# seqan/sahara

Measured on AMD Instinct MI355X. Metric: reads/s at k=2 edit, 10M×100bp vs 3Gbp index; achieved HBM GB/s, higher is better.
Workload: dtype u32; 1 GPU; C3: k=2 lev, 10000000x100bp reads (+RC) per GPU vs 3 Gbp 24-record index, h2-k2; reads_per_gpu=10000000, read_len=100, errors=2, ref_len=3000000000, records=24, generator=h2-k2, searches=3, parallelism=replicated-index x1 (query shards), hits_total=25990613, build_id=7339ec07fe5cacd5

## Files before the change

### include/sahara_hip.h

```cpp
#ifndef SAHARA_HIP_H
#define SAHARA_HIP_H

#include <stddef.h>
#include <stdint.h>

#ifdef __cplusplus
extern "C" {
#endif

typedef struct sahara_hit {
    uint64_t qid;
    uint32_t seq_id;
    uint32_t err;
    uint64_t pos;
} sahara_hit;

typedef struct sahara_index_info {
    uint32_t sigma;
    uint32_t sampling_rate;
    uint64_t n;
    uint64_t n_records;
    uint64_t n_samples;
    uint64_t device_bytes;
    uint32_t n_parts;
// ... 20 lines not shown
    double   text_ms;
    uint64_t fm_iterations;
    uint64_t text_iterations;
    uint64_t text_active;
    uint64_t text_refills;
    uint64_t text_cycles_refill;
    uint64_t text_cycles_step;
    uint64_t text_cycles_emit;
    uint64_t text_compare_steps;
    uint32_t text_grid;
    uint32_t pipelined;
    double   seed_ms;
    uint64_t text_steps;
    double   stage_ms;
    double   output_ms;
    uint64_t text_launches;
    uint64_t upload_chunks[3];
    uint64_t text_pos_tasks;
    uint64_t text_stolen;
    uint64_t best_rounds;
    uint64_t best_skipped;
    uint64_t reserved[6];
} sahara_stats;

const char* sahara_gpu_last_error(void);
int  sahara_gpu_device_count(void);
const char* sahara_build_id(void);

int  sahara_gpu_open(int device, const void* idx_image, size_t idx_bytes, void** ctx);
int  sahara_gpu_open_file(int device, const char* idx_path, void** ctx);
int  sahara_gpu_build(int device, const uint8_t* ranks, const uint64_t* rec_lens, uint64_t n_records,
                      uint32_t sigma, uint32_t sampling_rate, void** ctx);
int  sahara_gpu_save(void* ctx, const char* path);
int  sahara_gpu_index_info(void* ctx, sahara_index_info* info);
int  sahara_gpu_export(void* ctx, uint8_t* bwt_f, uint8_t* bwt_r, uint64_t* sampled_bits,
                       uint32_t* samples, uint64_t* C, uint64_t* rec_lens);
int  sahara_gpu_export_sa(void* ctx, uint32_t* sa);
int  sahara_gpu_export_text(void* ctx, uint8_t* text);
int  sahara_gpu_select_part(void* ctx, uint32_t part);
int  sahara_gpu_part_info(void* ctx, uint32_t part, sahara_index_info* info);
int  sahara_gpu_set_mode(void* ctx, int verify, int locate_sa);

int  sahara_gpu_search(void* ctx, const uint8_t* ranks, uint64_t n_patterns, uint32_t len,
                       const uint32_t* pi, const uint32_t* l, const uint32_t* u, uint32_t n_searches,
                       int edit, uint32_t max_hits, sahara_hit** hits, uint64_t* n_hits);
int  sahara_gpu_search_reads(void* ctx, const uint8_t* reads, uint64_t n_reads, uint32_t len, int reverse,
// ... 189 lines not shown
```

### sahara_amd/__init__.py

```python
from __future__ import annotations

import ctypes as C
import os

import numpy as np

__all__ = [
    "BiFMIndex", "HIT_DTYPE", "search", "search_reads", "search_reads_compact", "CompactHits", "PackedReads",
    "pack_reads", "search_packed", "search_packed_compact", "search_best", "search_best_reads", "search_best_packed",
    "search_best_packed_compact", "ALIGN_DTYPE", "ALIGN_MAX_ERR", "ALIGN_NONE", "align", "align_packed_compact",
    "align_stats", "cigar", "PAIR_SUMMARY_DTYPE", "PAIR_NONE", "PAIR_LINK_DTYPE", "LINK_PRIMARY", "pair_mapq", "read_fasta", "search_scheme", "scheme_parts",
    "scheme_generators",
    "scheme_counts", "synth_reference", "synth_reads", "interleave_rc", "load_fasta",
    "library_path", "lib", "SaharaError", "DNA5", "DNA4",
]

_HERE = os.path.dirname(os.path.abspath(__file__))
_LIB = None

DNA5 = {"sigma": 6, "chars": "$ACGNT"}
DNA4 = {"sigma": 5, "chars": "$ACGT"}

HIT_DTYPE = np.dtype([("qid", "<u8"), ("seq_id", "<u4"), ("err", "<u4"), ("pos", "<u8")])
ALIGN_MAX_ERR = 8
# ... 25 lines not shown
class IndexInfo(C.Structure):
    _fields_ = [("sigma", C.c_uint32), ("sampling_rate", C.c_uint32), ("n", C.c_uint64),
                ("n_records", C.c_uint64), ("n_samples", C.c_uint64), ("device_bytes", C.c_uint64),
                ("n_parts", C.c_uint32), ("kmer_depth", C.c_uint32)]


class Stats(C.Structure):
    _fields_ = [("patterns", C.c_uint64), ("batches", C.c_uint64), ("cursors", C.c_uint64),
                ("hits", C.c_uint64), ("search_ms", C.c_double), ("locate_ms", C.c_double),
                ("sort_ms", C.c_double), ("total_ms", C.c_double), ("nodes", C.c_uint64),
                ("rank_nodes", C.c_uint64), ("ext_lines", C.c_uint64), ("lf_steps", C.c_uint64),
                ("search_launches", C.c_uint32), ("search_grid", C.c_uint32),
                ("text_nodes", C.c_uint64), ("conversions", C.c_uint64), ("text_ms", C.c_double),
                ("fm_iterations", C.c_uint64), ("text_iterations", C.c_uint64), ("text_active", C.c_uint64),
                ("text_refills", C.c_uint64), ("text_cycles_refill", C.c_uint64),
                ("text_cycles_step", C.c_uint64), ("text_cycles_emit", C.c_uint64),
                ("text_compare_steps", C.c_uint64), ("text_grid", C.c_uint32), ("pipelined", C.c_uint32),
                ("seed_ms", C.c_double), ("text_steps", C.c_uint64), ("stage_ms", C.c_double),
                ("output_ms", C.c_double), ("text_launches", C.c_uint64),
                ("upload_chunks", C.c_uint64 * 3), ("text_pos_tasks", C.c_uint64),
                ("text_stolen", C.c_uint64), ("best_rounds", C.c_uint64), ("best_skipped", C.c_uint64),
                ("reserved", C.c_uint64 * 6)]

    def as_dict(self):
        return {n: (list(v) if isinstance(v, C.Array) else v) for n, v in
                ((n, getattr(self, n)) for n, _ in self._fields_)}


class AlignStats(C.Structure):
    _fields_ = [("hits", C.c_uint64), ("chunks", C.c_uint64), ("kernel_ms", C.c_double), ("stage_ms", C.c_double),
                ("total_ms", C.c_double)]


class LociStats(C.Structure):
    _fields_ = [("hits_in", C.c_uint64), ("loci", C.c_uint64), ("batches", C.c_uint64), ("kernel_ms", C.c_double)]


class PairsStats(C.Structure):
    _fields_ = [("hits_in", C.c_uint64), ("kept", C.c_uint64), ("pairs", C.c_uint64), ("batches", C.c_uint64),
                ("kernel_ms", C.c_double)]


class BestPairsStats(C.Structure):
    _fields_ = [("hits_in", C.c_uint64), ("kept", C.c_uint64), ("pairs", C.c_uint64), ("unique_pairs", C.c_uint64),
                ("batches", C.c_uint64), ("kernel_ms", C.c_double)]


PAIR_SUMMARY_DTYPE = np.dtype([("best", "u1"), ("next", "u1"), ("n_fwd", "<u2"), ("n_rev", "<u2"), ("reserved", "<u2")])
PAIR_NONE = 255
# ... 832 lines not shown
```

### sahara_amd/csrc/pass.cpp

```cpp
#include <algorithm>
#include <cstdlib>
#include <chrono>
#include <thread>

#include <sys/prctl.h>

#include "ctx.h"
#include "align_core.h"
#include "best_pairs_core.h"
#include "rescue_core.h"

namespace sahara {

DeviceIndex& partOf(Ctx* c, uint32_t p) { return p == 0 ? c->I : c->more.at(p - 1); }

void checkPairsCall(const Ctx* c, uint64_t npat, uint32_t len) {
    if (c->rescue.on) {
        if (!c->pairs.on) throw Error("rescue: needs pairs on (a mate is looked for in the pair rule's fragment window)");
        if (len > kAlignMaxLen)
            throw Error("rescue: the pattern length " + std::to_string(len) + " is above " + std::to_string(kAlignMaxLen));
        if (c->pairs.maxFrag >= len) {
            const PairDist d = pairDist(len, c->pairs.minFrag, c->pairs.maxFrag);
            if (d.dmax - d.dmin >= kRescueMaxWindow)
                throw Error("rescue: the fragment window of " + std::to_string(d.dmax - d.dmin + 1) +
// ... 41 lines not shown
                if (p) std::swap(c->I, c->more[p - 1]);
            });
            runOne(c, count);
        }
        if (c->outAll.cap < total + c->nout)
            c->outAll.growKeeping(std::max<uint64_t>((total + c->nout) + (total + c->nout) / 4, 1024), total, c->st);
        launchOffsetSeq(c->out.ptr, c->nout, c->partRec0[p], c->outAll.ptr + total, c->st);
        total += c->nout;
        const sahara_stats& S = c->stats;
        T.patterns = S.patterns;
        T.search_grid = S.search_grid;
        T.text_grid = S.text_grid;
        T.pipelined = S.pipelined;
        T.best_rounds = S.best_rounds;
        for (uint64_t sahara_stats::*f :
             {&sahara_stats::batches, &sahara_stats::cursors, &sahara_stats::nodes, &sahara_stats::rank_nodes,
              &sahara_stats::ext_lines, &sahara_stats::lf_steps, &sahara_stats::text_nodes,
              &sahara_stats::conversions, &sahara_stats::fm_iterations, &sahara_stats::text_iterations,
              &sahara_stats::text_active, &sahara_stats::text_refills, &sahara_stats::text_cycles_refill,
              &sahara_stats::text_cycles_step, &sahara_stats::text_cycles_emit, &sahara_stats::text_compare_steps,
              &sahara_stats::text_steps, &sahara_stats::text_launches,
              &sahara_stats::text_pos_tasks, &sahara_stats::text_stolen, &sahara_stats::best_skipped})
            T.*f += S.*f;
        for (double sahara_stats::*f : {&sahara_stats::search_ms, &sahara_stats::locate_ms, &sahara_stats::sort_ms,
                                        &sahara_stats::text_ms, &sahara_stats::seed_ms})
            T.*f += S.*f;
        T.search_launches += S.search_launches;
    }
    if (c->out.cap < total) {
        c->out.release();
        c->out.reserve(std::max<uint64_t>(total, 1024));
    }
    sortHitsByQid(c->outAll.ptr, total, c->npat, c->out.ptr, c->merge, c->tmp, c->st);
    SH_HIP(hipStreamSynchronize(c->st));
    c->sk.done = 0;
    c->nout = total;
    T.hits = total;
    T.total_ms = std::chrono::duration<double, std::milli>(std::chrono::steady_clock::now() - t0).count();
    T.stage_ms = c->stageMs;
    for (int b = 0; b < 3; ++b) T.upload_chunks[b] = c->stats.upload_chunks[b];
    c->stats = T;
}

void runOne(Ctx* c, bool count) {
    if (!c->sk.staged) throw Error("sahara_gpu_run: nothing staged");
    auto t0 = std::chrono::steady_clock::now();
// ... 184 lines not shown
    t.text3Bytes = (uint32_t)std::min<uint64_t>(text3Blocks(c->I.n) * 16, 0xFFFFFF00ull);
    t.pats3Bytes = (uint32_t)std::min<uint64_t>((P.bstart[b + 1] - q0) * c->patBlocks * 16, 0xFFFFFF00ull);
    t.m = c->m;
    t.nsearch = R.nsearch;
    t.table = reinterpret_cast<const uint2*>(c->cover.ptr + R.coverAt);
    t.tasks = sl.tasks.ptr;
    t.taskCount = sl.small.ptr + kSwTaskCount;
    t.taskBegin = r ? sl.small.ptr + kSwRoundTasks : nullptr;
    t.taskCap = c->taskCap;
    t.work = sl.queues.ptr + kQueueSeedTasks;
    t.hits = sl.hits.ptr;
    t.hitCap = c->hitCap;
    t.hitCount = sl.small.ptr + kSwHitCount;
    t.filled = sl.small.ptr + kSwFilled;
    t.flags = sl.small.ptr + kSwFlags;
    t.counters = c->counters.ptr;
    t.winBlocks = P.tx.winBlocks;
    t.exactWindow = P.tx.exactWindow ? 1u : 0u;
    t.stackCap = P.tx.textStack;
    t.tableWords = P.tx.tableWords;
    t.steps = P.k.textSteps;
    t.refillAt = P.k.refillAt;
    t.stealAt = P.k.stealAt;
    t.qcnt = sl.qcnt.ptr;
    t.rank = sl.rank.ptr;
    t.probe = P.probe ? 1u : 0u;
    t.isFirst = b == 0 && r == 0 ? 1u : 0u;
    return t;
}

enum : uint32_t { kLocFlags = 2, kLocSegCounts = 4 };

static LocateArgs locateArgs(Ctx* c, Ctx::Slot& sl, uint64_t nhits) {
    LocateArgs la{};
    la.hits = sl.hits.ptr;
    la.nhits = nhits;
    la.qoff = c->qoff.ptr;
    la.rank = sl.rank.ptr;
    la.occF = c->I.occF.ptr;
    for (int i = 0; i < 8; ++i) la.C[i] = (uint32_t)c->I.C[i];
    la.samples = c->I.samples.ptr;
    la.rate = c->I.rate;
    la.keys = c->k0.ptr;
    la.flags = c->small.ptr + kLocFlags;
    la.counters = c->counters.ptr + kCtLfSteps;
    la.sa = c->I.saFull.ptr;
// ... 351 lines not shown
            *total += ms;
            if (s == kStagePairs) c->stageStats.pairs.pairs += c->pinned.ptr[b].pairs;
            if (s == kStagePairs && c->pairs.linksOn && c->pairs.bufs.linkTimed) {
                SH_HIP(hipEventElapsedTime(&ms, c->pairs.bufs.linkStart, c->pairs.bufs.linkDone));
                c->stageStats.linkMs += ms;
            }
        }
        c->mark("checked", b);
    }
};

static void readCounters(Ctx* c, const PassPlan& P, sahara_stats& S, hipStream_t sC) {
    unsigned long long h[kCounters];
    auto per = [&](Counter sum, Counter n) { return (double)h[sum] / std::max(1.0, (double)h[n]); };
    if (P.probe) {
        SH_HIP(hipMemcpy(h, c->counters.ptr, sizeof(h), hipMemcpyDeviceToHost));
        auto since = [&](Counter i) { return (h[i] - h[kCtBornMin]) / 100.0; };
        std::fprintf(stderr, "text wave lives (first launch, us): last start %.1f first end %.1f last end %.1f mean %.1f; "
                     "tasks all taken seen first %.1f last %.1f by %llu waves, which ran on %.1f on average\n",
                     since(kCtBornMax), since(kCtEndMin), since(kCtEndMax),
                     h[kCtLifeSum] / 100.0 / std::max<double>(1, S.text_grid * 4.0), since(kCtDryMin), since(kCtDryMax),
                     h[kCtDryWaves], per(kCtDryRun, kCtDryWaves) / 100.0);
        std::fprintf(stderr, "text iterations before / after: %llu (busy lanes %.1f) / %llu (busy lanes %.1f); "
                     "nodes stolen %llu\n",
                     h[kCtIterPre], per(kCtActPre, kCtIterPre), h[kCtIterPost], per(kCtActPost, kCtIterPost), h[kCtStolen]);
        std::fprintf(stderr, "text wall per iteration (us) before: refill %.2f steps+emit %.2f; after: refill %.2f steps+emit %.2f\n",
                     per(kCtWallPreRefill, kCtIterPre) / 100.0, per(kCtWallPreStep, kCtIterPre) / 100.0,
                     per(kCtWallPostRefill, kCtIterPost) / 100.0, per(kCtWallPostStep, kCtIterPost) / 100.0);
    }
    SH_HIP(hipMemcpyAsync(h, c->counters.ptr, sizeof(h), hipMemcpyDeviceToHost, sC));
    SH_HIP(hipStreamSynchronize(sC));
    static const std::pair<uint64_t sahara_stats::*, Counter> statOf[] = {
        {&sahara_stats::nodes, kCtNodes}, {&sahara_stats::rank_nodes, kCtRankNodes},
        {&sahara_stats::ext_lines, kCtExtLines}, {&sahara_stats::lf_steps, kCtLfSteps},
        {&sahara_stats::text_nodes, kCtTextNodes}, {&sahara_stats::conversions, kCtTextTasks},
        {&sahara_stats::fm_iterations, kCtFmIter}, {&sahara_stats::text_iterations, kCtTextIter},
        {&sahara_stats::text_active, kCtTextActive}, {&sahara_stats::text_refills, kCtTextRefills},
        {&sahara_stats::text_cycles_refill, kCtCyRefill}, {&sahara_stats::text_cycles_step, kCtCyStep},
        {&sahara_stats::text_cycles_emit, kCtCyEmit}, {&sahara_stats::text_compare_steps, kCtCompareSteps},
        {&sahara_stats::text_steps, kCtTextSteps}, {&sahara_stats::text_pos_tasks, kCtPosTasks},
        {&sahara_stats::text_stolen, kCtStolen}, {&sahara_stats::best_skipped, kCtBestSkipped}};
    for (const auto& so : statOf) S.*so.first = h[so.second];
    if (P.k.dump) {
        for (uint32_t i = 0; i < kCounters; ++i) std::fprintf(stderr, "%s%llu", i ? " " : "counters ", h[i]);
        std::fprintf(stderr, "\n");
    }
}

void runPass(Ctx* c, bool count, bool redo, sahara_stats& S, bool& overflow) {
    const PassPlan P = makePlan(c, count, redo);
    const uint64_t nbatch = P.nbatch();
    overflow = false;
    S.patterns = c->npat;
    S.search_grid = P.blocks;
    S.text_grid = P.split ? P.textBlocks : 0u;
    S.pipelined = P.serial ? 0u : 1u;
    S.best_rounds = P.rounds > 1 ? P.rounds : 0u;
    c->stack.reserve((size_t)P.stackLevels * std::max(P.blocks, P.firstBlocks) * 256);
    initWorkCaps(c, P.maxBatch, P.k);
    c->pinned.reserve(nbatch);
    reserveLocate(c, P.maxBatch, Ctx::kSlots);
    for (auto& sl : c->slot) SH_HIP(hipMemsetAsync(sl.qcnt.ptr, 0, (P.maxBatch + 1) * sizeof(uint32_t), c->st));
    Pass ps{c, P, S, overflow, c->st, P.serial ? c->st : c->stB, P.serial ? c->st : c->stC, P.serial ? c->st : c->stD};
    auto syncAll = [&](std::initializer_list<hipStream_t> ss) {
        for (hipStream_t s : ss) SH_HIP(hipStreamSynchronize(s));
// ... 73 lines not shown
```

### sahara_amd/csrc/pass_plan.h

```cpp
#pragma once
#include <algorithm>
#include <cstdint>
#include <cstdlib>
#include <optional>
#include <vector>

#include "fm_step.h"

namespace sahara {

constexpr uint32_t kTextTableMin = 3u * 256u;

inline std::vector<uint64_t> parseRamp(const char* e) {
    std::vector<uint64_t> v;
    for (const char* p = e; p && *p;) {
        char* end = nullptr;
        const unsigned long long x = std::strtoull(p, &end, 10);
        if (end == p) break;
        if (x) v.push_back(x);
        p = (*end == ',' || *end == ':') ? end + 1 : end;
    }
    return v;
}

struct PassKnobs {
    bool pipeline, dump, chunkSeeds, kmerPos, seedTasks;
    uint32_t fmLdsDepth, fmStealAt, stealAt, split, textSteps, refillAt, pollUs;
    uint32_t hitCap, taskCap;
    unsigned long timerSlackNs;
    std::optional<long> batch, fmBpc, textBpc;
    std::vector<uint64_t> rampHead, rampTail;
};

inline PassKnobs readPassKnobs(bool verify) {
    auto num = [](const char* name) -> std::optional<long> {
        const char* e = std::getenv(name);
        return e ? std::optional<long>(std::atol(e)) : std::nullopt;
    };
    auto within = [](long lo, long v, long hi) { return std::max(lo, std::min(hi, v)); };
    PassKnobs k{};
    k.pipeline = num("SAHARA_PIPELINE").value_or(1) != 0;
    k.dump = std::getenv("SAHARA_DUMP_COUNTERS") != nullptr;
    k.fmLdsDepth = (uint32_t)within(0, num("SAHARA_FM_LDS_DEPTH").value_or(verify ? 0 : 4), 8);
    k.fmStealAt = (uint32_t)within(0, num("SAHARA_FM_STEAL_AT").value_or(verify ? 0 : 8), 64);
    k.stealAt = (uint32_t)within(0, num("SAHARA_STEAL_AT").value_or(8), 64);
    k.split = (uint32_t)std::max(0L, num("SAHARA_SPLIT").value_or(1));
    k.textSteps = (uint32_t)std::max(1L, num("SAHARA_TEXT_STEPS").value_or(2));
    k.refillAt = (uint32_t)within(1, num("SAHARA_REFILL_AT").value_or(8), 64);
    k.chunkSeeds = num("SAHARA_CHUNK_SEEDS").value_or(1) != 0;
    k.kmerPos = num("SAHARA_KMER_POS").value_or(1) != 0;
    k.seedTasks = num("SAHARA_SEED_TASKS").value_or(1) != 0;
    k.pollUs = (uint32_t)std::max(0L, num("SAHARA_POLL_US").value_or(20));
    k.timerSlackNs = (unsigned long)std::max(0L, num("SAHARA_TIMER_SLACK_NS").value_or(1000));
    if (auto v = num("SAHARA_HITCAP")) k.hitCap = (uint32_t)std::max(1L, *v);
    if (auto v = num("SAHARA_TASKCAP")) k.taskCap = (uint32_t)std::max(1L, *v);
    k.batch = num("SAHARA_BATCH");
    k.fmBpc = num("SAHARA_FM_BPC");
    k.textBpc = num("SAHARA_TEXT_BPC");
    k.rampHead = parseRamp(std::getenv("SAHARA_RAMP"));
    k.rampTail = parseRamp(std::getenv("SAHARA_RAMP_END"));
    return k;
}

inline uint64_t maxBatchOf(std::optional<long> batch, bool streaming, uint32_t nsearch, bool compactRecs,
                           uint64_t granularity = 1) {
    const uint64_t most = (1ull << 31) / nsearch;
    uint64_t mb = std::min<uint64_t>(streaming ? 1ull << 21 : 1ull << 22, most);
    if (batch) mb = std::max<uint64_t>(1, std::min<uint64_t>(most, (uint64_t)*batch));
// ... 94 lines not shown
```

### sahara_amd/csrc/search.h

```cpp
#pragma once
#include <hip/hip_runtime.h>

#include <cstddef>
#include <cstdint>

#include "../../include/sahara_hip.h"
#include "device_index.h"

namespace sahara {

struct SearchArgs {
    const OccLine* occF;
    const OccLine* occR;
    uint32_t C[8];
    uint32_t n;
    const uint32_t* pats;
    uint32_t patWords;
    uint32_t m;
    uint32_t nsearch;
    uint32_t nitems;
    const uint4* seeds;
    const uint32_t* seedItem;
    const uint32_t* seedCount;
    const uint32_t* scheme;
// ... 63 lines not shown
    uint64_t rows;
    uint32_t nbig, nhuge;
    uint64_t kept;
    uint64_t pairs;
};
static_assert(sizeof(BatchRecord) == 64 && offsetof(BatchRecord, slot) == 0 &&
              offsetof(BatchRecord, locateFlags) == 4 * 7 && offsetof(BatchRecord, rows) == 4 * kSlotWords &&
              offsetof(BatchRecord, nbig) == 4 * 10 && offsetof(BatchRecord, nhuge) == 4 * 11 &&
              offsetof(BatchRecord, kept) == 4 * 12, "BatchRecord is what kBatchTotals and the batch's stages write");

constexpr uint32_t kCounters = 56;
enum Counter : uint32_t {
    kCtNodes = 0, kCtRankNodes = 1, kCtExtLines = 2, kCtLfSteps = 3, kCtDigest = 4, kCtTextNodes = 5,
    kCtTextTasks = 6, kCtFmIter = 7, kCtTextIter = 8, kCtTextActive = 9, kCtTextRefills = 10,
    kCtCyRefill = 11, kCtCyStep = 12, kCtCyEmit = 13,
    kCtCompareSteps = 14, kCtTextSteps = 15,
    kCtPosTasks = 16,
    kCtBestSkipped = 17,
    kCtDryRun = 30, kCtDryWaves = 31,
    kCtBornMin = 33, kCtBornMax = 34, kCtEndMax = 35, kCtLifeSum = 36, kCtEndMin = 37,
    kCtDryMin = 38, kCtDryMax = 39,
    kCtIterPre = 40, kCtActPre = 41, kCtIterPost = 42, kCtActPost = 43,
    kCtStolen = 45,
    kCtWallPreRefill = 46, kCtWallPreStep = 47, kCtWallPostRefill = 48, kCtWallPostStep = 49
};
struct TextBatchArgs {
    const uint32_t* sa;
    const uint4* text3;
    const uint4* pats3;
    uint32_t patBlocks;
    uint32_t text3Bytes;
    uint32_t pats3Bytes;
    uint32_t m;
    uint32_t nsearch;
    const uint2* table;
    const uint4* tasks;
    const uint32_t* taskCount;
    const uint32_t* taskBegin;
    uint32_t taskCap;
    uint32_t* work;
    uint4* hits;
    uint32_t hitCap;
    uint32_t* hitCount;
    uint32_t* filled;
    uint32_t* flags;
    unsigned long long* counters;
    uint32_t winBlocks;
    uint32_t exactWindow;
    uint32_t stackCap;
    uint32_t tableWords;
    uint32_t steps;
    uint32_t refillAt;
    uint32_t stealAt;
    uint32_t* qcnt;
    uint32_t* rank;
    uint32_t probe;
    uint32_t isFirst;
};

struct LocateArgs {
    const uint4* hits;
    uint64_t nhits;
    const uint64_t* qoff;
    const uint32_t* rank;
    const OccLine* occF;
    uint32_t C[8];
    const uint32_t* samples;
    uint32_t rate;
    uint64_t* keys;
    uint32_t* flags;
    unsigned long long* counters;
    const uint32_t* sa;
    uint32_t useSA;
};

int searchBlocksPerCU(uint32_t sigma, bool edit, size_t lds);
// ... 123 lines not shown
```

### sahara_amd/csrc/search_device.h

```cpp
#pragma once
#include <hip/hip_runtime.h>

#include "search.h"

namespace sahara {
namespace {

#if defined(__HIP_DEVICE_COMPILE__)
#define GLOB(T, p) ((__attribute__((address_space(1))) T*)(p))
#else
#define GLOB(T, p) ((T*)(p))
#endif
typedef uint32_t U32x4 __attribute__((ext_vector_type(4)));
__device__ __forceinline__ uint4 loadGlobal4(const uint4* p) {
    const U32x4 v = *GLOB(const U32x4, p);
    return make_uint4(v.x, v.y, v.z, v.w);
}

constexpr uint32_t kSeedChunk = 64;
constexpr uint32_t kTaskChunk = 64;
static_assert(kTaskChunk >= 1 && kTaskChunk <= 64, "a chunk's records sit one per lane");
constexpr uint32_t kHitChunk = 64;

struct SlotRange {
    uint32_t next = 0, end = 0;
// ... 54 lines not shown
        __builtin_amdgcn_wave_barrier();
    }
};
__device__ __forceinline__ StealPlan stealPlan(bool thief, bool canGive, uint32_t stealAt, uint32_t lane,
                                               uint64_t ltMask) {
    const uint64_t I = __ballot(thief);
    const uint64_t D = __ballot(canGive);
    const uint32_t nI = (uint32_t)__popcll(I), nD = (uint32_t)__popcll(D);
    if (nI < stealAt || !nD) return {false, false, false, lane};
    const uint32_t n = min(nI, nD);
    const uint32_t r = (uint32_t)__popcll(I & ltMask);
    uint32_t donor = 0, rr = r;
    uint64_t dm = D;
#pragma unroll
    for (uint32_t w = 32; w; w >>= 1) {
        const uint32_t c = (uint32_t)__popcll(dm & ((1ull << w) - 1ull));
        if (rr >= c) { rr -= c; dm >>= w; donor += w; }
    }
    const bool takes = thief && r < n;
    const bool gives = ((D >> lane) & 1ull) && (uint32_t)__popcll(D & ltMask) < n;
    return {true, takes, gives, takes ? donor : lane};
}

constexpr uint32_t kLdsStarts = 256;
template <typename Starts>
__device__ __forceinline__ sahara_hit decodeKey(uint64_t k, uint64_t qid, const Starts& starts, uint32_t nrec) {
    const uint64_t gpos = k >> 4;
    uint32_t lo = 0, hi = nrec;
    while (hi - lo > 1) {
        const uint32_t mid = (lo + hi) >> 1;
        if (starts[mid] <= gpos) lo = mid; else hi = mid;
    }
    sahara_hit h;
    h.qid = qid;
    h.seq_id = lo;
    h.err = (uint32_t)(k & 15u);
    h.pos = gpos - starts[lo];
    return h;
}

struct HitLess {
    __host__ __device__ bool operator()(const sahara_hit& a, const sahara_hit& b) const {
        if (a.qid != b.qid) return a.qid < b.qid;
        if (a.seq_id != b.seq_id) return a.seq_id < b.seq_id;
        if (a.pos != b.pos) return a.pos < b.pos;
        return a.err < b.err;
// ... 6 lines not shown
```

### sahara_amd/csrc/search_text.hip

```cpp

#include <hip/hip_runtime.h>

#include "fm_step.h"
#include "search_device.h"
#include "text_step.h"

namespace sahara {
namespace {

__device__ __forceinline__ uint32_t read32(const uint32_t* A, int o, uint32_t b) {
    const int i = o >> 5;
    return __builtin_amdgcn_alignbit(A[(3 * i + 3 + (int)b) * 256], A[(3 * i + (int)b) * 256], (uint32_t)o & 31u);
}
__device__ __forceinline__ Planes chain32(const uint32_t* A, uint32_t o, bool fwd) {
    const int off = (int)o - (fwd ? 0 : 32);
    Planes r;
    uint32_t v[3];
#pragma unroll
    for (uint32_t b = 0; b < 3; ++b) {
        const uint32_t w = read32(A, off, b);
        v[b] = fwd ? w : __builtin_bitreverse32(w);
    }
    r.b0 = v[0]; r.b1 = v[1]; r.b2 = v[2];
    return r;
// ... 157 lines not shown
    const StealPlan p = stealPlan(!ln.have && ln.sp == 0u, ln.sp >= 2u || (ln.sp == 1u && ln.have), stealAt, lane, ltMask);
    if (!p.any) return false;
    const uint32_t dPid = __shfl(ln.pid, p.donor), dWb = __shfl(ln.wb, p.donor), dBase = __shfl(ln.sBase, p.donor);
    const uint32_t dTid = (threadIdx.x & ~63u) | p.donor;
    if (p.takes) {
        const uint32_t* src = L.slot + dTid;
        uint32_t* dst = L.slot + threadIdx.x;
        for (uint32_t k = 0; k < L.copyWords(); ++k) dst[k * 256u] = src[k * 256u];
        const uint2 node = reinterpret_cast<const uint2*>(L.slot + L.copyWords() * 256u)[dTid];
        ln.cur = {node.x, node.y};
        ln.pid = dPid;
        ln.wb = dWb;
        ln.sBase = dBase;
        ln.have = true;
    }
    p.settle();
    if (p.gives) {
        for (uint32_t d = 1; d < ln.sp; ++d) L.stackPut(d - 1u, L.stackGet(d));
        --ln.sp;
    }
    return p.takes;
}

struct HitWriter {
    SlotRange slots;
    uint32_t rankSlot = ~0u, rankVal = 0;
    uint32_t filled = 0;
    __device__ __forceinline__ void emit(const TextBatchArgs& a, bool leaf, uint32_t lane, uint64_t ltMask, uint32_t pid,
                                         uint32_t pos, uint32_t e) {
        uint32_t s;
        if (slots.take(leaf, lane, ltMask, a.hitCount, s) && leaf) {
            if (s < a.hitCap) {
                a.hits[s] = make_uint4(pid, pos, 1u, e | kPosKnown);
                if (rankSlot != ~0u) a.rank[rankSlot] = rankVal;
                rankVal = atomicAdd(a.qcnt + pid, 1u);
                rankSlot = s;
            } else {
                atomicOr(a.flags, kFlagHits);
            }
            ++filled;
        }
    }
    __device__ __forceinline__ void finish(const TextBatchArgs& a, uint32_t lane) {
        slots.close(lane, a.hits, a.hitCap);
        if (rankSlot != ~0u) a.rank[rankSlot] = rankVal;
        if (filled) atomicAdd(a.filled, filled);
    }
};

template <bool COUNT>
struct TextProbe {
    __device__ __forceinline__ TextProbe(const TextBatchArgs&, uint32_t, uint64_t*) {}
    __device__ __forceinline__ void iterBegin() {}
    __device__ __forceinline__ void refilled(bool, bool, bool) {}
    __device__ __forceinline__ void stolen(bool) {}
    __device__ __forceinline__ void stepped(const TextStepResult&) {}
    __device__ __forceinline__ void stepsDone() {}
    __device__ __forceinline__ void emitted(bool) {}
    __device__ __forceinline__ void flush() {}
};
template <>
struct TextProbe<true> {
    const TextBatchArgs& a;
    const uint32_t lane;
    const bool wall;
    uint64_t* born;
    uint64_t cNodes = 0, cCmp = 0, cSteps = 0, cSteal = 0;
    uint64_t tIter = 0, tActive = 0, tRefill = 0;
    uint64_t cyRefill = 0, cyStep = 0, cyEmit = 0, t0 = 0;
    uint32_t pIterPre = 0, pIterPost = 0, pActPre = 0, pActPost = 0;
    uint64_t pwPreA = 0, pwPreB = 0, pwPostA = 0, pwPostB = 0, pw0 = 0, pw1 = 0;

    __device__ __forceinline__ TextProbe(const TextBatchArgs& args, uint32_t l, uint64_t* waveClock)
        : a(args), lane(l), wall(args.probe != 0u), born(waveClock + 2u * (threadIdx.x >> 6)) {
        if (wall && lane == 0) born[0] = wall_clock64(), born[1] = 0;
    }
    __device__ __forceinline__ void iterBegin() {
        if (wall) pw0 = wall_clock64();
        t0 = clock64();
    }
    __device__ __forceinline__ void refilled(bool qDone, bool active, bool refill) {
        const uint32_t act = (uint32_t)__popcll(__ballot(active));
        if (wall) {
            if (qDone && lane == 0 && born[1] == 0) born[1] = wall_clock64();
            if (qDone) { ++pIterPost; pActPost += act; } else { ++pIterPre; pActPre += act; }
            pw1 = wall_clock64();
        }
        if (lane == 0) { ++tIter; tActive += act; tRefill += refill ? 1u : 0u; }
        const uint64_t t1 = clock64();
        cyRefill += t1 - t0;
        t0 = t1;
    }
    __device__ __forceinline__ void stolen(bool took) { cSteal += took ? 1u : 0u; }
    __device__ __forceinline__ void stepped(const TextStepResult& r) {
        cNodes += r.nodes;
        cCmp += r.compares;
        cSteps += r.steps;
    }
    __device__ __forceinline__ void stepsDone() {
        const uint64_t t1 = clock64();
        cyStep += t1 - t0;
        t0 = t1;
    }
    __device__ __forceinline__ void emitted(bool qDone) {
        cyEmit += clock64() - t0;
        if (wall) {
            const uint64_t pw2 = wall_clock64();
            if (qDone) { pwPostA += pw1 - pw0; pwPostB += pw2 - pw1; }
            else { pwPreA += pw1 - pw0; pwPreB += pw2 - pw1; }
        }
    }
    __device__ __forceinline__ void add(uint32_t counter, uint64_t v) {
        atomicAdd(a.counters + counter, (unsigned long long)v);
    }
    __device__ __forceinline__ void flush() {
        if (wall && a.isFirst && lane == 0) {
// ... 10 lines not shown
                add(kCtDryWaves, 1);
            }
            add(kCtIterPre, pIterPre);
            add(kCtActPre, pActPre);
            add(kCtIterPost, pIterPost);
            add(kCtActPost, pActPost);
            add(kCtWallPreRefill, pwPreA);
            add(kCtWallPreStep, pwPreB);
            add(kCtWallPostRefill, pwPostA);
            add(kCtWallPostStep, pwPostB);
        }
        add(kCtTextNodes, cNodes);
        if (lane == 0) {
            add(kCtTextIter, tIter);
            add(kCtTextActive, tActive);
            add(kCtTextRefills, tRefill);
            add(kCtCyRefill, cyRefill);
            add(kCtCyStep, cyStep);
            add(kCtCyEmit, cyEmit);
        }
        add(kCtCompareSteps, cCmp);
        add(kCtTextSteps, cSteps);
        if (cSteal) add(kCtStolen, cSteal);
    }
};

template <bool EDIT, bool COUNT, int SHAPE>
__global__ __launch_bounds__(256) void kSearchTextBatch(TextBatchArgs a) {
    extern __shared__ uint32_t lds[];
    uint2* SC = reinterpret_cast<uint2*>(lds);
    for (uint32_t i = threadIdx.x; i < a.nsearch * a.m; i += blockDim.x) SC[i] = a.table[i];
    __syncthreads();

    const uint32_t lane = threadIdx.x & 63u;
    const uint64_t ltMask = (1ull << lane) - 1ull;
    constexpr TextShape kShape = textShape(SHAPE);
    LaneLds L;
    L.table = SC;
    L.slot = lds + a.tableWords;
    L.winBlocks = SHAPE ? kShape.win : a.winBlocks;
    L.patBlocks = SHAPE ? kShape.pat : a.patBlocks;
    L.exactWindow = SHAPE ? kShape.exact : a.exactWindow != 0u;
    L.W = L.slot + threadIdx.x;
    L.P = L.slot + 3u * L.winBlocks * 256u + threadIdx.x;
    L.S = reinterpret_cast<uint2*>(L.slot + L.copyWords() * 256u) + threadIdx.x;
    const uint32_t winLen = L.winBlocks * 32u;
    const __amdgpu_buffer_rsrc_t textBuf = bufferOf(a.text3, a.text3Bytes);
    const __amdgpu_buffer_rsrc_t patBuf = bufferOf(a.pats3, a.pats3Bytes);
    const uint32_t m = a.m;
    const uint32_t tEnd = min(*a.taskCount, a.taskCap);
    const uint32_t tBase = a.taskBegin ? min(*a.taskBegin, tEnd) : 0u;

    TextLane ln;
    bool exhausted = false, bad = false;
// ... 3 lines not shown
    TextProbe<COUNT> probe(a, lane, waveClock);

    for (;;) {
        probe.iterBegin();
        const bool idle = !ln.have && ln.sp == 0 && !exhausted;
        const uint64_t idleMask = __ballot(idle);
        const bool busy = __any(ln.busy());
        const bool refill = !busy || __popcll(idleMask) >= a.refillAt;
        const bool need = refill && idle;
        uint64_t pending = refill ? idleMask : 0ull;
        if (pending) feed.resolveNext(lane);
        while (pending) {
            if (feed.chunkEmpty()) {
                if (!feed.haveNext) break;
                feed.advance(lane);
                if (feed.chunkEmpty()) continue;
            }
            uint4 t;
            const bool mine = feed.take(pending, lane, ltMask, t);
            if (mine && t.y != 0u) startTask(ln, t, L, m, textBuf, patBuf);
            pending &= ~__ballot(mine);
        }
        if (feed.dry() && need && !ln.have) exhausted = true;
        if (a.stealAt && feed.dry()) probe.stolen(stealStage(ln, L, a.stealAt, lane, ltMask));
        if (!__any(ln.busy() || (!exhausted && !feed.dry()))) break;
        probe.refilled(feed.qDone, ln.busy(), refill);

        bool leaf = false;
        uint32_t leafStart = 0, leafE = 0;
        for (uint32_t step = 0; step < a.steps; ++step) {
            const bool pop = !ln.have && !leaf && ln.sp > 0;
            const TextNode top = L.stackGet(pop ? ln.sp - 1u : 0u);
            if (pop) { ln.cur = top; --ln.sp; ln.have = true; }
            const bool live = ln.have && !leaf;
            if (!__any(live)) break;

            const TextStepResult r = textStep<EDIT>(
                ln.cur, ln.sp, live, a.stackCap, m, winLen, [&](uint32_t p) { return L.row(ln.sBase + p); },
                [&](uint32_t o, bool fwd) { return chain32(L.P, o, fwd); },
                [&](uint32_t o, bool fwd) { return chain32(L.W, o, fwd); },
                [&](uint32_t d, const TextNode& n) { L.stackPut(d, n); });
            ln.cur = r.cur;
            ln.sp = r.sp;
            ln.have = live ? r.have : ln.have;
            if (r.leaf) { leaf = true; leafStart = r.leafStart; leafE = r.leafE; }
            bad = bad || r.bad;
            probe.stepped(r);
        }
        probe.stepsDone();
        hits.emit(a, leaf, lane, ltMask, ln.pid, ln.wb + leafStart, leafE);
        probe.emitted(feed.qDone);
    }
    probe.flush();
    hits.finish(a, lane);
    if (__any(bad) && lane == 0) atomicOr(a.flags, kFlagTextStack);
}

const void* textBatchKernel(bool edit, bool count, int shape) {
#define SH_ROW(E, C) {(const void*)kSearchTextBatch<E, C, 0>, (const void*)kSearchTextBatch<E, C, 1>, \
                      (const void*)kSearchTextBatch<E, C, 2>}
    static const void* const kernels[2][2][kTextShapes] = {{SH_ROW(false, false), SH_ROW(false, true)},
                                                            {SH_ROW(true, false), SH_ROW(true, true)}};
#undef SH_ROW
    return kernels[edit][count][shape];
}

}

int textShapeOf(uint32_t winBlocks, uint32_t patBlocks, bool exactWindow) {
    for (int shape = 1; shape < kTextShapes; ++shape) {
        const TextShape t = textShape(shape);
        if (winBlocks == t.win && patBlocks == t.pat && exactWindow == t.exact) return shape;
    }
    return 0;
// ... 16 lines not shown
```

Baseline: 997.9 million reads/s.

## Add wave retirement with cross-wave orphan adoption in text search tail

Adds a tail phase to the text search kernel. Once the feed runs dry, a wave with few busy lanes publishes their lane state to LDS and exits, and idle lanes in other waves of the workgroup adopt that state and copy the window and stack. The aim is to cut the long tail where mostly idle waves keep occupying the SIMD. The mechanism is disabled by default (SAHARA_RETIRE_AT=0), but the change also adds an amdgpu_waves_per_eu attribute to the kernel. It also extracts the step loop into a function, adds a static LDS box and new counters.

```diff
diff --git a/include/sahara_hip.h b/include/sahara_hip.h
--- a/include/sahara_hip.h
+++ b/include/sahara_hip.h
@@ -66,6 +66,11 @@
     uint64_t best_skipped;
     uint64_t reserved[6];
 } sahara_stats;
+enum sahara_stats_reserved {
+    SAHARA_STAT_TEXT_RETIRED = 0,
+    SAHARA_STAT_TEXT_PUBLISHED = 1,
+    SAHARA_STAT_TEXT_ADOPTED = 2
+};
 
 const char* sahara_gpu_last_error(void);
 int  sahara_gpu_device_count(void);
diff --git a/sahara_amd/__init__.py b/sahara_amd/__init__.py
--- a/sahara_amd/__init__.py
+++ b/sahara_amd/__init__.py
@@ -71,9 +71,13 @@
                 ("text_stolen", C.c_uint64), ("best_rounds", C.c_uint64), ("best_skipped", C.c_uint64),
                 ("reserved", C.c_uint64 * 6)]
 
+    IN_RESERVED = ("text_retired", "text_published", "text_adopted")
+
     def as_dict(self):
-        return {n: (list(v) if isinstance(v, C.Array) else v) for n, v in
-                ((n, getattr(self, n)) for n, _ in self._fields_)}
+        d = {n: (list(v) if isinstance(v, C.Array) else v) for n, v in
+             ((n, getattr(self, n)) for n, _ in self._fields_)}
+        d.update(zip(self.IN_RESERVED, d["reserved"]))
+        return d
 
 
 class AlignStats(C.Structure):
diff --git a/sahara_amd/csrc/pass.cpp b/sahara_amd/csrc/pass.cpp
--- a/sahara_amd/csrc/pass.cpp
+++ b/sahara_amd/csrc/pass.cpp
@@ -87,6 +87,8 @@
               &sahara_stats::text_steps, &sahara_stats::text_launches,
               &sahara_stats::text_pos_tasks, &sahara_stats::text_stolen, &sahara_stats::best_skipped})
             T.*f += S.*f;
+        for (int i : {SAHARA_STAT_TEXT_RETIRED, SAHARA_STAT_TEXT_PUBLISHED, SAHARA_STAT_TEXT_ADOPTED})
+            T.reserved[i] += S.reserved[i];
         for (double sahara_stats::*f : {&sahara_stats::search_ms, &sahara_stats::locate_ms, &sahara_stats::sort_ms,
                                         &sahara_stats::text_ms, &sahara_stats::seed_ms})
             T.*f += S.*f;
@@ -317,6 +319,7 @@
     t.steps = P.k.textSteps;
     t.refillAt = P.k.refillAt;
     t.stealAt = P.k.stealAt;
+    t.retireAt = P.k.retireAt;
     t.qcnt = sl.qcnt.ptr;
     t.rank = sl.rank.ptr;
     t.probe = P.probe ? 1u : 0u;
@@ -714,8 +717,9 @@
                      h[kCtLifeSum] / 100.0 / std::max<double>(1, S.text_grid * 4.0), since(kCtDryMin), since(kCtDryMax),
                      h[kCtDryWaves], per(kCtDryRun, kCtDryWaves) / 100.0);
         std::fprintf(stderr, "text iterations before / after: %llu (busy lanes %.1f) / %llu (busy lanes %.1f); "
-                     "nodes stolen %llu\n",
-                     h[kCtIterPre], per(kCtActPre, kCtIterPre), h[kCtIterPost], per(kCtActPost, kCtIterPost), h[kCtStolen]);
+                     "nodes stolen %llu; waves retired %llu nodes adopted %llu\n",
+                     h[kCtIterPre], per(kCtActPre, kCtIterPre), h[kCtIterPost], per(kCtActPost, kCtIterPost), h[kCtStolen],
+                     h[kCtRetired], h[kCtAdopted]);
         std::fprintf(stderr, "text wall per iteration (us) before: refill %.2f steps+emit %.2f; after: refill %.2f steps+emit %.2f\n",
                      per(kCtWallPreRefill, kCtIterPre) / 100.0, per(kCtWallPreStep, kCtIterPre) / 100.0,
                      per(kCtWallPostRefill, kCtIterPost) / 100.0, per(kCtWallPostStep, kCtIterPost) / 100.0);
@@ -733,6 +737,9 @@
         {&sahara_stats::text_steps, kCtTextSteps}, {&sahara_stats::text_pos_tasks, kCtPosTasks},
         {&sahara_stats::text_stolen, kCtStolen}, {&sahara_stats::best_skipped, kCtBestSkipped}};
     for (const auto& so : statOf) S.*so.first = h[so.second];
+    S.reserved[SAHARA_STAT_TEXT_RETIRED] = h[kCtRetired];
+    S.reserved[SAHARA_STAT_TEXT_PUBLISHED] = h[kCtPublished];
+    S.reserved[SAHARA_STAT_TEXT_ADOPTED] = h[kCtAdopted];
     if (P.k.dump) {
         for (uint32_t i = 0; i < kCounters; ++i) std::fprintf(stderr, "%s%llu", i ? " " : "counters ", h[i]);
         std::fprintf(stderr, "\n");
diff --git a/sahara_amd/csrc/pass_plan.h b/sahara_amd/csrc/pass_plan.h
--- a/sahara_amd/csrc/pass_plan.h
+++ b/sahara_amd/csrc/pass_plan.h
@@ -23,9 +23,11 @@
     return v;
 }
 
+constexpr long kRetireAtDefault = 0;
+
 struct PassKnobs {
     bool pipeline, dump, chunkSeeds, kmerPos, seedTasks;
-    uint32_t fmLdsDepth, fmStealAt, stealAt, split, textSteps, refillAt, pollUs;
+    uint32_t fmLdsDepth, fmStealAt, stealAt, retireAt, split, textSteps, refillAt, pollUs;
     uint32_t hitCap, taskCap;
     unsigned long timerSlackNs;
     std::optional<long> batch, fmBpc, textBpc;
@@ -44,6 +46,7 @@
     k.fmLdsDepth = (uint32_t)within(0, num("SAHARA_FM_LDS_DEPTH").value_or(verify ? 0 : 4), 8);
     k.fmStealAt = (uint32_t)within(0, num("SAHARA_FM_STEAL_AT").value_or(verify ? 0 : 8), 64);
     k.stealAt = (uint32_t)within(0, num("SAHARA_STEAL_AT").value_or(8), 64);
+    k.retireAt = (uint32_t)within(0, num("SAHARA_RETIRE_AT").value_or(kRetireAtDefault), 64);
     k.split = (uint32_t)std::max(0L, num("SAHARA_SPLIT").value_or(1));
     k.textSteps = (uint32_t)std::max(1L, num("SAHARA_TEXT_STEPS").value_or(2));
     k.refillAt = (uint32_t)within(1, num("SAHARA_REFILL_AT").value_or(8), 64);
diff --git a/sahara_amd/csrc/retire_plan.h b/sahara_amd/csrc/retire_plan.h
--- /dev/null
+++ b/sahara_amd/csrc/retire_plan.h
@@ -0,0 +1,42 @@
+#pragma once
+#include <cstdint>
+
+#ifndef SAHARA_HD
+#if defined(__HIPCC__)
+#define SAHARA_HD __host__ __device__ __forceinline__
+#else
+#define SAHARA_HD inline
+#endif
+#endif
+
+namespace sahara {
+
+SAHARA_HD uint32_t nthSetBit(uint64_t mask, uint32_t r) {
+    uint32_t at = 0;
+    for (uint32_t w = 32; w; w >>= 1) {
+        const uint32_t c = (uint32_t)__builtin_popcountll(mask & ((1ull << w) - 1ull));
+        if (r >= c) { r -= c; mask >>= w; at += w; }
+    }
+    return at;
+}
+
+SAHARA_HD bool mayRetire(uint64_t busy, uint32_t retireAt, uint32_t lanes = 64) {
+    const uint32_t nb = (uint32_t)__builtin_popcountll(busy);
+    return nb >= 1u && nb <= retireAt && nb <= lanes - nb;
+}
+
+struct OrphanAt { uint32_t source, state; };
+SAHARA_HD OrphanAt orphanAt(uint64_t busy, uint32_t r, uint32_t lanes = 64) {
+    const uint64_t all = lanes >= 64u ? ~0ull : (1ull << lanes) - 1ull;
+    return {nthSetBit(busy, r), nthSetBit(~busy & all, r)};
+}
+
+SAHARA_HD bool claimedOrphan(uint32_t c, uint64_t idle, uint32_t lane, uint32_t n, uint32_t& orphan) {
+    if (!((idle >> lane) & 1ull)) return false;
+    orphan = c + (uint32_t)__builtin_popcountll(idle & ((1ull << lane) - 1ull));
+    return orphan < n;
+}
+
+SAHARA_HD bool mayLeave(uint32_t aliveBefore) { return aliveBefore >= 2u; }
+
+}
diff --git a/sahara_amd/csrc/search.h b/sahara_amd/csrc/search.h
--- a/sahara_amd/csrc/search.h
+++ b/sahara_amd/csrc/search.h
@@ -109,7 +109,8 @@
     kCtDryMin = 38, kCtDryMax = 39,
     kCtIterPre = 40, kCtActPre = 41, kCtIterPost = 42, kCtActPost = 43,
     kCtStolen = 45,
-    kCtWallPreRefill = 46, kCtWallPreStep = 47, kCtWallPostRefill = 48, kCtWallPostStep = 49
+    kCtWallPreRefill = 46, kCtWallPreStep = 47, kCtWallPostRefill = 48, kCtWallPostStep = 49,
+    kCtRetired = 50, kCtPublished = 51, kCtAdopted = 52
 };
 struct TextBatchArgs {
     const uint32_t* sa;
@@ -139,6 +140,7 @@
     uint32_t steps;
     uint32_t refillAt;
     uint32_t stealAt;
+    uint32_t retireAt;
     uint32_t* qcnt;
     uint32_t* rank;
     uint32_t probe;
diff --git a/sahara_amd/csrc/search_device.h b/sahara_amd/csrc/search_device.h
--- a/sahara_amd/csrc/search_device.h
+++ b/sahara_amd/csrc/search_device.h
@@ -1,6 +1,7 @@
 #pragma once
 #include <hip/hip_runtime.h>
 
+#include "retire_plan.h"
 #include "search.h"
 
 namespace sahara {
@@ -101,6 +102,15 @@
     return {true, takes, gives, takes ? donor : lane};
 }
 
+struct RetireBox {
+    uint64_t busy[4];
+    uint32_t published[4];
+    uint32_t claimed[4];
+    uint32_t alive;
+    uint32_t lastLooks;
+};
+static_assert(sizeof(RetireBox) <= 128, "the text geometry leaves ~190 B of static LDS at m = 672 with three searches");
+
 constexpr uint32_t kLdsStarts = 256;
 template <typename Starts>
 __device__ __forceinline__ sahara_hit decodeKey(uint64_t k, uint64_t qid, const Starts& starts, uint32_t nrec) {
diff --git a/sahara_amd/csrc/search_text.hip b/sahara_amd/csrc/search_text.hip
--- a/sahara_amd/csrc/search_text.hip
+++ b/sahara_amd/csrc/search_text.hip
@@ -203,6 +203,100 @@
     return p.takes;
 }
 
+constexpr uint32_t kTextWaves = 4;
+__device__ __forceinline__ uint32_t coldTid() {
+    uint32_t t = threadIdx.x;
+    asm volatile("" : "+v"(t));
+    return t;
+}
+__device__ __forceinline__ uint32_t boxLoad(const uint32_t* p) {
+    return __hip_atomic_load(p, __ATOMIC_ACQUIRE, __HIP_MEMORY_SCOPE_WORKGROUP);
+}
+__device__ __forceinline__ bool leaveBox(RetireBox& box, uint32_t lane, bool ending) {
+    uint32_t old = 0;
+    if (lane == 0) {
+        old = __hip_atomic_fetch_sub(&box.alive, 1u, __ATOMIC_ACQ_REL, __HIP_MEMORY_SCOPE_WORKGROUP);
+        if (!mayLeave(old)) {
+            __hip_atomic_fetch_add(&box.alive, 1u, __ATOMIC_RELAXED, __HIP_MEMORY_SCOPE_WORKGROUP);
+            if (ending) __hip_atomic_store(&box.lastLooks, 1u, __ATOMIC_RELAXED, __HIP_MEMORY_SCOPE_WORKGROUP);
+        }
+    }
+    return mayLeave(__shfl(old, 0));
+}
+constexpr uint32_t kOrphanWords = 6;
+static_assert(kOrphanWords <= 3u * 2u, "an idle lane's window and pattern hold an orphan's state");
+
+__device__ __forceinline__ bool adoptStage(TextLane& ln, const LaneLds& L, RetireBox& box, uint32_t lane,
+                                           uint64_t ltMask) {
+    bool took = false;
+    const uint32_t tid = coldTid(), self = tid >> 6;
+#pragma nounroll
+    for (uint32_t w = 0; w < kTextWaves; ++w) {
+        const uint64_t idle = __ballot(!ln.busy());
+        if (!idle) break;
+        if (w == self) continue;
+        const uint32_t n = boxLoad(&box.published[w]);
+        if (!n || boxLoad(&box.claimed[w]) >= n) continue;
+        uint32_t c = 0;
+        if (lane == 0)
+            c = __hip_atomic_fetch_add(&box.claimed[w], (uint32_t)__popcll(idle), __ATOMIC_RELAXED,
+                                       __HIP_MEMORY_SCOPE_WORKGROUP);
+        c = __shfl(c, 0);
+        uint32_t o = 0;
+        if (claimedOrphan(c, idle, lane, n, o)) {
+            const uint32_t* rec = L.slot + (w * 64u + orphanAt(box.busy[w], o).state);
+            const uint32_t srcTid = (rec[512] >> 16) & 0xFFu;
+            const uint32_t* src = L.slot + srcTid;
+            uint32_t* dst = L.slot + tid;
+            ln.cur = {rec[0], rec[256]};
+            ln.sp = rec[512] & 0xFFFFu;
+            ln.have = (rec[512] >> 31) != 0u;
+            ln.pid = rec[768];
+            ln.wb = rec[1024];
+            ln.sBase = rec[1280];
+#pragma nounroll
+            for (uint32_t k = 0; k < L.copyWords(); ++k) dst[k * 256u] = src[k * 256u];
+            const uint2* stack = reinterpret_cast<const uint2*>(L.slot + L.copyWords() * 256u) + srcTid;
+            uint2* mine = reinterpret_cast<uint2*>(L.slot + L.copyWords() * 256u) + tid;
+#pragma nounroll
+            for (uint32_t d = 0; d < ln.sp; ++d) mine[d * 256u] = stack[d * 256u];
+            took = true;
+        }
+    }
+    return took;
+}
+
+__device__ __forceinline__ bool retireStage(TextLane& ln, const LaneLds& L, RetireBox& box, uint32_t retireAt,
+                                            uint32_t lane, uint64_t ltMask, uint32_t& left) {
+    const uint64_t B = __ballot(ln.busy());
+    if (!mayRetire(B, retireAt) || boxLoad(&box.alive) < 2u) return false;
+    const uint32_t tid = coldTid(), wave = tid >> 6, n = (uint32_t)__popcll(B), r = (uint32_t)__popcll(B & ltMask);
+    if (ln.busy()) {
+        uint32_t* rec = L.slot + ((tid & ~63u) | orphanAt(B, r).state);
+        rec[0] = ln.cur.x;
+        rec[256] = ln.cur.y;
+        rec[512] = ln.sp | (tid << 16) | (ln.have ? 1u << 31 : 0u);
+        rec[768] = ln.pid;
+        rec[1024] = ln.wb;
+        rec[1280] = ln.sBase;
+    }
+    if (lane == 0) box.busy[wave] = B;
+    __builtin_amdgcn_fence(__ATOMIC_RELEASE, "workgroup");
+    if (lane == 0) __hip_atomic_store(&box.published[wave], n, __ATOMIC_RELEASE, __HIP_MEMORY_SCOPE_WORKGROUP);
+    if (leaveBox(box, lane, false)) {
+        left = n;
+        return true;
+    }
+    const uint32_t taken = min(boxLoad(&box.claimed[wave]), n);
+    left = taken;
+    if (ln.busy() && r < taken) {
+        ln.have = false;
+        ln.sp = 0;
+    }
+    if (lane == 0) __hip_atomic_store(&box.published[wave], 0u, __ATOMIC_RELAXED, __HIP_MEMORY_SCOPE_WORKGROUP);
+    return false;
+}
+
 struct HitWriter {
     SlotRange slots;
     uint32_t rankSlot = ~0u, rankVal = 0;
@@ -235,6 +329,8 @@
     __device__ __forceinline__ void iterBegin() {}
     __device__ __forceinline__ void refilled(bool, bool, bool) {}
     __device__ __forceinline__ void stolen(bool) {}
+    __device__ __forceinline__ void adopted(bool) {}
+    __device__ __forceinline__ void retired(bool, uint32_t) {}
     __device__ __forceinline__ void stepped(const TextStepResult&) {}
     __device__ __forceinline__ void stepsDone() {}
     __device__ __forceinline__ void emitted(bool) {}
@@ -246,7 +342,8 @@
     const uint32_t lane;
     const bool wall;
     uint64_t* born;
-    uint64_t cNodes = 0, cCmp = 0, cSteps = 0, cSteal = 0;
+    uint64_t cNodes = 0, cCmp = 0, cSteps = 0, cSteal = 0, cAdopt = 0;
+    uint32_t cRetired = 0, cLeft = 0;
     uint64_t tIter = 0, tActive = 0, tRefill = 0;
     uint64_t cyRefill = 0, cyStep = 0, cyEmit = 0, t0 = 0;
     uint32_t pIterPre = 0, pIterPost = 0, pActPre = 0, pActPost = 0;
@@ -273,6 +370,10 @@
         t0 = t1;
     }
     __device__ __forceinline__ void stolen(bool took) { cSteal += took ? 1u : 0u; }
+    __device__ __forceinline__ void adopted(bool took) { cAdopt += took ? 1u : 0u; }
+    __device__ __forceinline__ void retired(bool went, uint32_t left) {
+        if (lane == 0) { cRetired += went ? 1u : 0u; cLeft += left; }
+    }
     __device__ __forceinline__ void stepped(const TextStepResult& r) {
         cNodes += r.nodes;
         cCmp += r.compares;
@@ -329,14 +430,52 @@
         add(kCtCompareSteps, cCmp);
         add(kCtTextSteps, cSteps);
         if (cSteal) add(kCtStolen, cSteal);
+        if (cAdopt) add(kCtAdopted, cAdopt);
+        if (cRetired) add(kCtRetired, cRetired);
+        if (cLeft) add(kCtPublished, cLeft);
     }
 };
 
+template <bool EDIT, typename Probe>
+__device__ __forceinline__ void stepStage(const TextBatchArgs& a, TextLane& ln, const LaneLds& L, uint32_t m,
+                                          uint32_t winLen, HitWriter& hits, bool& bad, Probe& probe, uint32_t lane,
+                                          uint64_t ltMask, bool qDone) {
+    bool leaf = false;
+    uint32_t leafStart = 0, leafE = 0;
+    for (uint32_t step = 0; step < a.steps; ++step) {
+        const bool pop = !ln.have && !leaf && ln.sp > 0;
+        const TextNode top = L.stackGet(pop ? ln.sp - 1u : 0u);
+        if (pop) { ln.cur = top; --ln.sp; ln.have = true; }
+        const bool live = ln.have && !leaf;
+        if (!__any(live)) break;
+
+        const TextStepResult r = textStep<EDIT>(
+            ln.cur, ln.sp, live, a.stackCap, m, winLen, [&](uint32_t p) { return L.row(ln.sBase + p); },
+            [&](uint32_t o, bool fwd) { return chain32(L.P, o, fwd); },
+            [&](uint32_t o, bool fwd) { return chain32(L.W, o, fwd); },
+            [&](uint32_t d, const TextNode& n) { L.stackPut(d, n); });
+        ln.cur = r.cur;
+        ln.sp = r.sp;
+        ln.have = live ? r.have : ln.have;
+        if (r.leaf) { leaf = true; leafStart = r.leafStart; leafE = r.leafE; }
+        bad = bad || r.bad;
+        probe.stepped(r);
+    }
+    probe.stepsDone();
+    hits.emit(a, leaf, lane, ltMask, ln.pid, ln.wb + leafStart, leafE);
+    probe.emitted(qDone);
+}
+
+constexpr unsigned textWavesPerSimd(bool count, int shape) { return (shape == 1 ? 5u : 4u) - (count ? 1u : 0u); }
 template <bool EDIT, bool COUNT, int SHAPE>
-__global__ __launch_bounds__(256) void kSearchTextBatch(TextBatchArgs a) {
+__global__ __launch_bounds__(256) __attribute__((amdgpu_waves_per_eu(textWavesPerSimd(COUNT, SHAPE))))
+void kSearchTextBatch(TextBatchArgs a) {
     extern __shared__ uint32_t lds[];
     uint2* SC = reinterpret_cast<uint2*>(lds);
     for (uint32_t i = threadIdx.x; i < a.nsearch * a.m; i += blockDim.x) SC[i] = a.table[i];
+    __shared__ RetireBox box;
+    if (threadIdx.x < kTextWaves) box.published[threadIdx.x] = 0u, box.claimed[threadIdx.x] = 0u;
+    if (threadIdx.x == 0) box.alive = kTextWaves, box.lastLooks = 0u;
     __syncthreads();
 
     const uint32_t lane = threadIdx.x & 63u;
@@ -386,34 +525,30 @@
             pending &= ~__ballot(mine);
         }
         if (feed.dry() && need && !ln.have) exhausted = true;
-        if (a.stealAt && feed.dry()) probe.stolen(stealStage(ln, L, a.stealAt, lane, ltMask));
+        if (feed.dry()) {
+            if (a.retireAt) break;
+            if (a.stealAt) probe.stolen(stealStage(ln, L, a.stealAt, lane, ltMask));
+        }
         if (!__any(ln.busy() || (!exhausted && !feed.dry()))) break;
         probe.refilled(feed.qDone, ln.busy(), refill);
-
-        bool leaf = false;
-        uint32_t leafStart = 0, leafE = 0;
-        for (uint32_t step = 0; step < a.steps; ++step) {
-            const bool pop = !ln.have && !leaf && ln.sp > 0;
-            const TextNode top = L.stackGet(pop ? ln.sp - 1u : 0u);
-            if (pop) { ln.cur = top; --ln.sp; ln.have = true; }
-            const bool live = ln.have && !leaf;
-            if (!__any(live)) break;
-
-            const TextStepResult r = textStep<EDIT>(
-                ln.cur, ln.sp, live, a.stackCap, m, winLen, [&](uint32_t p) { return L.row(ln.sBase + p); },
-                [&](uint32_t o, bool fwd) { return chain32(L.P, o, fwd); },
-                [&](uint32_t o, bool fwd) { return chain32(L.W, o, fwd); },
-                [&](uint32_t d, const TextNode& n) { L.stackPut(d, n); });
-            ln.cur = r.cur;
-            ln.sp = r.sp;
-            ln.have = live ? r.have : ln.have;
-            if (r.leaf) { leaf = true; leafStart = r.leafStart; leafE = r.leafE; }
-            bad = bad || r.bad;
-            probe.stepped(r);
-        }
-        probe.stepsDone();
-        hits.emit(a, leaf, lane, ltMask, ln.pid, ln.wb + leafStart, leafE);
-        probe.emitted(feed.qDone);
+        stepStage<EDIT>(a, ln, L, m, winLen, hits, bad, probe, lane, ltMask, feed.qDone);
+    }
+    if (a.retireAt && feed.dry()) {
+        for (;;) {
+            probe.iterBegin();
+            probe.adopted(adoptStage(ln, L, box, lane, ltMask));
+            uint32_t left = 0;
+            const bool went = retireStage(ln, L, box, a.retireAt, lane, ltMask, left);
+            probe.retired(went, left);
+            if (went) break;
+            if (a.stealAt) probe.stolen(stealStage(ln, L, a.stealAt, lane, ltMask));
+            if (!__any(ln.busy())) {
+                if (boxLoad(&box.lastLooks) || leaveBox(box, lane, true)) break;
+                continue;
+            }
+            probe.refilled(true, ln.busy(), false);
+            stepStage<EDIT>(a, ln, L, m, winLen, hits, bad, probe, lane, ltMask, true);
+        }
     }
     probe.flush();
     hits.finish(a, lane);
```

New measurement: 996.5 million reads/s, median of 2. No clear change (-0.1%).
